# patrikhuber/superviseddescent

Measured on NVIDIA H100. Metric: faces/sec RCR 22-landmark detect, higher is better.
Workload: dtype f32

## Files before the change

### superviseddescent_b200/csrc/sd_hog.cu

```cuda
#include "sd_internal.cuh"
#include "sd_hog_common.cuh"

#include <cmath>
#include <cuda_pipeline.h>

namespace {

constexpr int kHogThreads = 256;

struct HogArgs {
    const uint8_t* images;
    int width, height, row_stride;
    long long image_stride;
    int image_count;
    const int* image_index;
    const sd_roi* roi;
    const sd_frame* frames;
    uint8_t* roi_miss;
    const float* x;
    long long ldx;
    int N, L;
    int variant, nc, cs, K, fs, dd;
    const int* half;
    HogOrient orient;
    const int* rtab;
    const float* btab;
    int tma_count;
    float* A;
    long long ld;
    int* geometry;
    uint8_t* patches;
    int8_t* bins;
    int* status;
};

__device__ __forceinline__ int clip_index(int x, int a, int b) { return x >= a ? (x < b ? x : b - 1) : a; }
__device__ __forceinline__ short sat_short(int v) { return (short)(v > 32767 ? 32767 : (v < -32768 ? -32768 : v)); }

__global__ void hog_geometry_kernel(const float* __restrict__ x, long long ldx, int N, int L, const sd_eyes_dev eyes, float rel,
                                    int fixed_half, int fs, int* __restrict__ half_out, int* __restrict__ rtab, int* __restrict__ status)
{
    const int i = blockIdx.x;
    if (i >= N) return;
    __shared__ int s_half;
    if (threadIdx.x == 0) {
        bool degenerate;
        const int half = sd_patch_half(x + (long long)i * ldx, L, eyes, rel, fixed_half, &degenerate);
        if (degenerate) atomicOr(status, 1);
        half_out[i] = half;
        s_half = half;
    }
    __syncthreads();
    const int P = 2 * s_half;
    int* rt = rtab + (long long)i * 5 * fs;
    for (int t = threadIdx.x; t < fs; t += blockDim.x) {
        const double inv_scale = __ddiv_rn((double)fs, (double)P);
        const double scale = __ddiv_rn(1.0, inv_scale);
        float f = (float)__dadd_rn(__dmul_rn((double)t + 0.5, scale), -0.5);
        const int s = (int)floorf(f);
        f = __fsub_rn(f, (float)s);
        int sx = s;
        float fx = f;
        if (sx < 0) { fx = 0.f; sx = 0; }
        if (sx >= P - 1) { fx = 0.f; sx = P - 1; }
        const short2 xa = make_short2(sat_short(__float2int_rn(__fmul_rn(__fsub_rn(1.f, fx), 2048.f))),
                                      sat_short(__float2int_rn(__fmul_rn(fx, 2048.f))));
        const short2 yb = make_short2(sat_short(__float2int_rn(__fmul_rn(__fsub_rn(1.f, f), 2048.f))),
                                      sat_short(__float2int_rn(__fmul_rn(f, 2048.f))));
        rt[t] = sx;
        rt[fs + t] = *reinterpret_cast<const int*>(&xa);
        rt[2 * fs + t] = clip_index(s, 0, P);
        rt[3 * fs + t] = clip_index(s + 1, 0, P);
        rt[4 * fs + t] = *reinterpret_cast<const int*>(&yb);
    }
}

__global__ void hog_bintab_kernel(int fs, int nc, int cs, float* __restrict__ btab)
{
    __shared__ int s_sbin[256];
    for (int t = threadIdx.x; t < fs; t += blockDim.x) {
        int b;
        float w1, w2;
        hog_spatial_weight(t, cs, &b, &w1, &w2);
        s_sbin[t] = b;
        for (int c = 0; c < nc; ++c) btab[c * fs + t] = (b == c) ? w1 : ((b == c - 1) ? w2 : 0.f);
    }
    __syncthreads();
    int* lohi = reinterpret_cast<int*>(btab + nc * fs);
    for (int c = threadIdx.x; c < nc; c += blockDim.x) {
        int lo = fs, hi = -1;
        for (int t = 1; t <= fs - 2; ++t) {
            const int b = s_sbin[t];
            if (b == c || b == c - 1) { if (t < lo) lo = t; hi = t; }
        }
        lohi[c] = lo;
        lohi[nc + c] = hi;
    }
}

struct HogSmem {
    int patch, bin, r1, xofs, yofs0, yofs1, xa, yb, wcell, lo, hi, vote, mbar, stage_end, total;
    int tpad;
};

__host__ __device__ inline int align_up(int v, int a) { return (v + a - 1) / a * a; }

__host__ __device__ inline HogSmem hog_smem_layout(int fs, int nc, int K)
{
    HogSmem s;
    int o = 0;
    s.patch = o;
    o = align_up(fs * fs, 16);
    s.xofs = o;   o += fs * 4;
    s.yofs0 = o;  o += fs * 4;
    s.yofs1 = o;  o += fs * 4;
    s.xa = o;     o += fs * 4;
    s.yb = o;     o += fs * 4;
    s.wcell = o;  o += nc * fs * 4;
    s.lo = o;     o += nc * 4;
    s.hi = o;     o += nc * 4;
    s.mbar = align_up(o, 8); o = s.mbar + 8;
    o = align_up(o, 128);
    s.bin = o;    o = align_up(o + fs * fs, 16);
    s.r1 = o;     o = align_up(o + fs * fs * 4, 16);
    s.tpad = align_up((fs - 2) * nc, 32);
    s.vote = o;
    o += 2 * K * s.tpad * 4;
    s.stage_end = o;
    s.total = align_up(o, 16);
    return s;
}

constexpr int kTmaClasses = 8;
__host__ __device__ constexpr int hog_tma_box(int c) { return c == 0 ? 32 : c == 1 ? 48 : c == 2 ? 64 : c == 3 ? 80 : c == 4 ? 96 : c == 5 ? 112 : c == 6 ? 128 : 160; }
struct HogMaps { CUtensorMap m[kTmaClasses]; };

template <int KT, int NCT, int CST, int NT>
__global__ void __launch_bounds__(NT, NCT > 0 ? 2048 / NT : 0) hog_patch_kernel(const __grid_constant__ HogArgs a, const __grid_constant__ HogMaps maps)
{
    static_assert(NT % 32 == 0 && NT >= 64, "hog_patch_kernel needs whole warps and at least 64 threads");
    constexpr int kWarps = NT / 32;
    extern __shared__ __align__(128) unsigned char smem[];
    const int K = KT > 0 ? KT : a.K;
    const int nc = NCT > 0 ? NCT : a.nc;
    const int fs = (NCT > 0 && CST > 0) ? NCT * CST : a.fs;
    const int cells = nc * nc;
    const HogSmem lay = hog_smem_layout(fs, nc, K);
    uint8_t* s_patch = smem + lay.patch;
    int8_t* s_bin = reinterpret_cast<int8_t*>(smem + lay.bin);
    float* s_gmag = reinterpret_cast<float*>(smem + lay.r1);
    int* s_xofs = reinterpret_cast<int*>(smem + lay.xofs);
    int* s_yofs0 = reinterpret_cast<int*>(smem + lay.yofs0);
    int* s_yofs1 = reinterpret_cast<int*>(smem + lay.yofs1);
    short2* s_xa = reinterpret_cast<short2*>(smem + lay.xa);
    short2* s_yb = reinterpret_cast<short2*>(smem + lay.yb);
    float* s_wcell = reinterpret_cast<float*>(smem + lay.wcell);
    int* s_lo = reinterpret_cast<int*>(smem + lay.lo);
    int* s_hi = reinterpret_cast<int*>(smem + lay.hi);
    float* s_T = reinterpret_cast<float*>(smem + lay.vote);
    uint64_t* s_mbar = reinterpret_cast<uint64_t*>(smem + lay.mbar);

    const int tid = threadIdx.x;
    const int lane = tid & 31, warp = tid >> 5;
    const long long patch_id = blockIdx.x;
    const int sample = (int)(patch_id / a.L);
    const int lm = (int)(patch_id - (long long)sample * a.L);

    const float* __restrict__ row = a.x + (long long)sample * a.ldx;
    const int half = __ldg(a.half + sample);
    const int P = 2 * half;
    const int cx = __float2int_rn(row[lm]);
    const int cy = __float2int_rn(row[lm + a.L]);
    int img_idx = a.image_index ? a.image_index[sample] : sample;
    if (img_idx < 0 || img_idx >= a.image_count) {
        img_idx = 0;
        if (tid == 0 && a.status) atomicOr(a.status, 2);
    }
    int W = a.width, H = a.height, rs = a.row_stride;
    const uint8_t* __restrict__ img = a.images + (long long)img_idx * a.image_stride;
    if (a.frames) {
        const sd_frame f = a.frames[img_idx];
        W = f.width; H = f.height; rs = f.row_stride;
        img = a.images + f.offset;
    }
    int rx = 0, ry = 0, rw = W, rh = H;
    if (a.roi) {
        const sd_roi r = a.roi[img_idx];
        rx = r.x; ry = r.y; rw = r.w; rh = r.h; rs = r.row_stride;
        img = a.images + r.offset;
    }
    if (tid == 0 && a.geometry) {
        a.geometry[patch_id * 3 + 0] = cx;
        a.geometry[patch_id * 3 + 1] = cy;
        a.geometry[patch_id * 3 + 2] = half;
    }

    const int x0 = cx - half, y0 = cy - half;
    uint8_t* s_stage = smem + lay.bin;
    const int stage_cap = lay.stage_end - lay.bin;
    int tma_box = 0;
    const int tma_shift = x0 & 15;
#pragma unroll
    for (int c = kTmaClasses - 1; c >= 0; --c)
        if (c < a.tma_count && hog_tma_box(c) >= P + tma_shift && hog_tma_box(c) * hog_tma_box(c) <= stage_cap) tma_box = hog_tma_box(c);
    if (tma_box > 0 && tid == 0) {
        int cls = 0;
#pragma unroll
        for (int c = 0; c < kTmaClasses; ++c) if (hog_tma_box(c) == tma_box) cls = c;
        hog_tma_load(s_mbar, s_stage, &maps.m[cls], x0 - tma_shift, y0, img_idx, tma_box * tma_box);
    }

    {
        const int* __restrict__ rt = a.rtab + (long long)sample * 5 * fs;
        for (int t = tid; t < fs; t += NT) {
            s_xofs[t] = __ldg(rt + t);
            const int xa = __ldg(rt + fs + t), yb = __ldg(rt + 4 * fs + t);
            s_xa[t] = *reinterpret_cast<const short2*>(&xa);
            s_yofs0[t] = __ldg(rt + 2 * fs + t);
            s_yofs1[t] = __ldg(rt + 3 * fs + t);
            s_yb[t] = *reinterpret_cast<const short2*>(&yb);
        }
        for (int i = tid; i < nc * fs; i += NT) s_wcell[i] = __ldg(a.btab + i);
        const int* __restrict__ lohi = reinterpret_cast<const int*>(a.btab + nc * fs);
        if (tid < nc) { s_lo[tid] = __ldg(lohi + tid); s_hi[tid] = __ldg(lohi + nc + tid); }
    }
    {
        const bool resident = x0 >= rx && y0 >= ry && x0 + P <= rx + rw && y0 + P <= ry + rh && x0 >= 0 && y0 >= 0 && x0 + P <= W && y0 + P <= H;
        const uintptr_t align_bits = reinterpret_cast<uintptr_t>(img) | (uintptr_t)rs;
        const bool vec16 = !tma_box && resident && (align_bits & 15) == 0;
        const bool words = !tma_box && resident && (align_bits & 3) == 0;
        const int shiftb = tma_box ? tma_shift : (vec16 ? ((x0 - rx) & 15) : (words ? ((x0 - rx) & 3) : 0));
        const int pitch = tma_box ? tma_box : ((P + 15 + 15) & ~15);
        const bool staged = pitch * P <= stage_cap;
        bool miss = false;
        if (staged) {
            if (tma_box) {
            } else if (vec16) {
                const int nvec = (shiftb + P + 15) >> 4;
                const int gs = nvec <= 8 ? 3 : (nvec <= 16 ? 4 : 5);
                const int lv = lane & ((1 << gs) - 1), lr = lane >> gs, rows_per_pass = 32 >> gs;
                const uint8_t* wrow = img + (long long)(y0 - ry) * rs + (x0 - rx - shiftb);
                for (int r = warp * rows_per_pass + lr; r < P; r += kWarps * rows_per_pass)
                    for (int v = lv; v < nvec; v += (1 << gs))
                        reinterpret_cast<uint4*>(s_stage + r * pitch)[v] = __ldg(reinterpret_cast<const uint4*>(wrow + (long long)r * rs) + v);
            } else if (words) {
                const int nwords = (shiftb + P + 3) >> 2;
                const uint8_t* wrow = img + (long long)(y0 - ry) * rs + (x0 - rx - shiftb);
                for (int r = warp; r < P; r += kWarps) {
                    const uint32_t* src = reinterpret_cast<const uint32_t*>(wrow + (long long)r * rs);
                    uint32_t* dst = reinterpret_cast<uint32_t*>(s_stage + r * pitch);
                    for (int w = lane; w < nwords; w += 32) dst[w] = __ldg(src + w);
                }
            } else {
                for (int r = warp; r < P; r += kWarps) {
                    const int iy = y0 + r;
                    const bool rowin = (unsigned)iy < (unsigned)H;
                    const bool rowres = iy >= ry && iy < ry + rh;
                    for (int c = lane; c < P; c += 32) {
                        const int ix = x0 + c;
                        int v = 0;
                        if (rowin && (unsigned)ix < (unsigned)W) {
                            if (rowres && ix >= rx && ix < rx + rw) v = __ldg(img + (long long)(iy - ry) * rs + (ix - rx));
                            else miss = true;
                        }
                        s_stage[r * pitch + c] = (uint8_t)v;
                    }
                }
            }
            __syncthreads();
            if (tma_box) hog_tma_wait(s_mbar);
            if (fs <= 64) {
                const int groups = NT / fs;
                const int dx = tid % fs, g = tid / fs;
                if (g < groups) {
                    const int sx = s_xofs[dx];
                    const int sx1 = min(sx + 1, P - 1);
                    const int ax = s_xa[dx].x, bx = s_xa[dx].y;
                    const uint8_t* base = s_stage + shiftb;
#pragma unroll 4
                    for (int dy = g; dy < fs; dy += groups) {
                        const short2 yb = s_yb[dy];
                        const uint8_t* r0 = base + s_yofs0[dy] * pitch;
                        const uint8_t* r1 = base + s_yofs1[dy] * pitch;
                        const int t0 = (int)r0[sx] * ax + (int)r0[sx1] * bx;
                        const int t1 = (int)r1[sx] * ax + (int)r1[sx1] * bx;
                        const int v = ((((int)yb.x * (t0 >> 4)) >> 16) + (((int)yb.y * (t1 >> 4)) >> 16) + 2) >> 2;
                        s_patch[dy * fs + dx] = (uint8_t)v;
                    }
                }
            } else {
                for (int dy = warp; dy < fs; dy += kWarps) {
                    const short2 yb = s_yb[dy];
                    const uint8_t* r0 = s_stage + s_yofs0[dy] * pitch + shiftb;
                    const uint8_t* r1 = s_stage + s_yofs1[dy] * pitch + shiftb;
                    for (int dx = lane; dx < fs; dx += 32) {
                        const int sx = s_xofs[dx];
                        const int sx1 = min(sx + 1, P - 1);
                        const short2 xa = s_xa[dx];
                        const int t0 = (int)r0[sx] * xa.x + (int)r0[sx1] * xa.y;
                        const int t1 = (int)r1[sx] * xa.x + (int)r1[sx1] * xa.y;
                        const int v = ((((int)yb.x * (t0 >> 4)) >> 16) + (((int)yb.y * (t1 >> 4)) >> 16) + 2) >> 2;
                        s_patch[dy * fs + dx] = (uint8_t)v;
                    }
                }
            }
        } else {
            __syncthreads();
            for (int dy = warp; dy < fs; dy += kWarps) {
                const short2 yb = s_yb[dy];
                const int iy0 = y0 + s_yofs0[dy], iy1 = y0 + s_yofs1[dy];
                for (int dx = lane; dx < fs; dx += 32) {
                    const int sx = s_xofs[dx];
                    const short2 xa = s_xa[dx];
                    int p[4];
#pragma unroll
                    for (int q = 0; q < 4; ++q) {
                        const int ix = x0 + sx + (q & 1), iy = (q & 2) ? iy1 : iy0;
                        int v = 0;
                        if ((q & 1) && xa.y == 0) { p[q] = 0; continue; }
                        if ((unsigned)ix < (unsigned)W && (unsigned)iy < (unsigned)H) {
                            if (ix >= rx && ix < rx + rw && iy >= ry && iy < ry + rh) v = __ldg(img + (long long)(iy - ry) * rs + (ix - rx));
                            else miss = true;
                        }
                        p[q] = v;
                    }
                    const int t0 = p[0] * xa.x + p[1] * xa.y;
                    const int t1 = p[2] * xa.x + p[3] * xa.y;
                    const int v = ((((int)yb.x * (t0 >> 4)) >> 16) + (((int)yb.y * (t1 >> 4)) >> 16) + 2) >> 2;
                    s_patch[dy * fs + dx] = (uint8_t)v;
                }
            }
        }
        if (miss && a.roi_miss) a.roi_miss[img_idx] = 1;
        if (a.patches) {
            __syncthreads();
            for (int i = tid; i < fs * fs; i += NT) a.patches[patch_id * fs * fs + i] = s_patch[i];
        }
    }
    __syncthreads();

    {
        const int iw = fs - 2, npix = iw * iw;
        for (int i = tid; i < npix; i += NT) {
            const int y = i / iw, x = i - y * iw;
            const int idx = (y + 1) * fs + (x + 1);
            const int gx = (int)s_patch[idx + 1] - (int)s_patch[idx - 1];
            const int gy = (int)s_patch[idx + fs] - (int)s_patch[idx - fs];
            const int g2 = gx * gx + gy * gy;
            const float g = __fsqrt_rn((float)g2);
            const int b = hog_bin(a.orient, K, gx, gy, g);
            s_bin[idx] = (int8_t)b;
            s_gmag[idx] = b < 0 ? 0.f : g;
        }
    }
    if (a.bins) {
        __syncthreads();
        for (int idx = tid; idx < fs * fs; idx += NT) {
            const int y = idx / fs, x = idx - y * fs;
            const bool interior = x >= 1 && x <= fs - 2 && y >= 1 && y <= fs - 2;
            a.bins[patch_id * fs * fs + idx] = interior ? s_bin[idx] : (int8_t)-1;
        }
    }
    if (!a.A) return;
    __syncthreads();

    {
        const int nrow = fs - 2, ntask = nrow * nc, tpad = lay.tpad;
        for (int task = tid; task < ntask; task += NT) {
            const int ci = task / nrow, y = 1 + task - ci * nrow;
            const int xlo = s_lo[ci], xhi = s_hi[ci];
            const int8_t* bp = s_bin + y * fs + xlo;
            const float* gp = s_gmag + y * fs + xlo;
            const float* wp = s_wcell + ci * fs + xlo;
            float* T = s_T + task;
            for (int b = 0; b < 2 * K; ++b) T[b * tpad] = 0.f;
#pragma unroll 2
            for (int x = xlo; x <= xhi; ++x) {
                const int b = max((int)*bp++, 0);
                float* q = T + b * tpad;
                *q = __fadd_rn(*q, __fmul_rn(*gp++, *wp++));
            }
        }
        __syncthreads();
        float* __restrict__ out = a.A + (long long)sample * a.ld + (long long)lm * cells * a.dd;
        for (int i = tid; i < 2 * K * cells; i += NT) {
            const int b = i / cells, c = i - b * cells;
            const int cj = c / nc, ci = c - cj * nc;
            const int ylo = s_lo[cj], yhi = s_hi[cj];
            const float* Tp = s_T + b * tpad + ci * nrow + (ylo - 1);
            const float* wy = s_wcell + cj * fs + ylo;
            float acc = 0.f;
            for (int y = ylo; y <= yhi; ++y) acc = __fadd_rn(acc, __fmul_rn(*Tp++, *wy++));
            out[i] = acc;
        }
    }
}

struct NormArgs {
    float* A;
    long long ld;
    int N, L, nc, K, dd, variant, per_cta;
};

__host__ __device__ inline int hog_norm_smem(int nc, int K, int per_cta)
{
    const int cells = nc * nc;
    return per_cta * (8 + 2 * K * cells * 4 + cells * 8 + (nc + 1) * (nc + 1) * 8);
}

template <int KT>
__global__ void __launch_bounds__(kHogThreads) hog_normalise_kernel(const NormArgs a)
{
    extern __shared__ __align__(16) unsigned char s_norm[];
    const int K = KT > 0 ? KT : a.K;
    const int nc = a.nc, nb = nc + 1, cells = nc * nc, blocks = nb * nb, hsz = 2 * K * cells, per_lm = cells * a.dd;
    const long long first = (long long)blockIdx.x * a.per_cta;
    const int np = (int)min((long long)a.per_cta, (long long)a.N * a.L - first);
    long long* s_slice = reinterpret_cast<long long*>(s_norm);
    double* s_energy = reinterpret_cast<double*>(s_slice + a.per_cta);
    double* s_fac = s_energy + a.per_cta * cells;
    float* s_hist = reinterpret_cast<float*>(s_fac + a.per_cta * blocks);
    for (int p = threadIdx.x; p < np; p += kHogThreads) {
        const long long id = first + p;
        const int sample = (int)(id / a.L), lm = (int)(id - (long long)sample * a.L);
        s_slice[p] = (long long)sample * a.ld + (long long)lm * per_lm;
        if (lm == 0) a.A[(long long)sample * a.ld + (long long)a.L * per_lm] = 1.0f;
    }
    __syncthreads();
    for (int i = threadIdx.x; i < np * hsz; i += kHogThreads) {
        const int p = i / hsz;
        __pipeline_memcpy_async(s_hist + i, a.A + s_slice[p] + (i - p * hsz), sizeof(float));
    }
    __pipeline_commit();
    __pipeline_wait_prior(0);
    __syncthreads();
    for (int i = threadIdx.x; i < np * cells; i += kHogThreads) {
        const int p = i / cells, c = i - p * cells;
        s_energy[i] = (double)hog_cell_energy(s_hist + p * hsz + c, cells, K);
    }
    __syncthreads();
    for (int i = threadIdx.x; i < np * blocks; i += kHogThreads) {
        const int p = i / blocks, j = i - p * blocks;
        const int jy = j / nb, jx = j - jy * nb;
        s_fac[i] = hog_block_factor(s_energy + p * cells, nc, max(jx - 1, 0), min(jx, nc - 1), max(jy - 1, 0), min(jy, nc - 1));
    }
    __syncthreads();
    for (int i = threadIdx.x; i < np * cells; i += kHogThreads) {
        const int p = i / cells, c = i - p * cells;
        const int cj = c / nc, ci = c - cj * nc;
        const double* F = s_fac + p * blocks + cj * nb + ci;
        const double fac[4] = {F[0], F[1], F[nb], F[nb + 1]};
        float* __restrict__ out = a.A + s_slice[p] + ci * nc + cj;
        hog_cell_features(fac, s_hist + p * hsz + c, cells, K, a.variant, [=](int d, float v) { out[d * cells] = v; });
    }
}

int launch_hog(sd_ctx* ctx, const sd_image_batch* images, const int32_t* d_image_index, const float* d_x,
               int64_t ldx, int N, int L, const sd_normalisation* eyes, const sd_hog_param* p, float* d_A,
               int64_t ld, int32_t* d_geometry, uint8_t* d_patches, int8_t* d_bins)
{
    SD_REQUIRE(ctx, images && images->d_data && d_x && p, "null argument");
    SD_REQUIRE(ctx, N >= 0 && L >= 1, "bad sample / landmark count");
    SD_REQUIRE(ctx, p->variant == 0 || p->variant == 1, "unknown HOG variant");
    SD_REQUIRE(ctx, p->num_bins >= 1 && p->num_bins <= SD_MAX_BINS, "num_bins must be in [1,16]");
    SD_REQUIRE(ctx, p->num_cells >= 1 && p->cell_size >= 1, "bad cell configuration");
    const int fs = p->num_cells * p->cell_size;
    SD_REQUIRE(ctx, fs > 3 && fs <= 256, "resized patch must be 4..256 px (hog.c:545-546 asserts > 3)");
    SD_REQUIRE(ctx, (fs + p->cell_size / 2) / p->cell_size == p->num_cells, "hogWidth != num_cells");
    SD_REQUIRE(ctx, ldx >= 2 * L, "ldx < 2L");
    if (N == 0) return SD_OK;
    const bool fixed = !eyes || eyes->kind == 0;
    int fixed_half = 0;
    if (fixed) {
        fixed_half = p->num_cells * (p->cell_size / 2);
        SD_REQUIRE(ctx, 2 * fixed_half == fs, "the fixed-patch HogTransform needs an even cell_size (patch == num_cells * cell_size)");
    } else if (eyes->kind != 1) {
        return sd_fail(ctx, SD_ERR_INVALID, "unknown normalisation kind");
    }

    HogArgs a;
    sd_eyes_dev eyes_dev;
    memset(&eyes_dev, 0, sizeof(eyes_dev));
    int rc = fixed ? SD_OK : sd_eyes_to_dev(ctx, eyes, L, &eyes_dev);
    if (rc) return rc;
    a.images = images->d_data;
    a.width = images->width; a.height = images->height; a.row_stride = images->row_stride;
    a.image_stride = images->image_stride; a.image_count = images->count;
    a.image_index = d_image_index;
    a.roi = images->d_roi;
    a.roi_miss = images->d_roi_miss;
    a.frames = images->d_frames;
    if (!d_image_index) SD_REQUIRE(ctx, images->count >= N, "fewer images than samples and no image index");
    a.x = d_x; a.ldx = ldx; a.N = N; a.L = L;
    a.variant = p->variant; a.nc = p->num_cells; a.cs = p->cell_size; a.K = p->num_bins; a.fs = fs;
    a.dd = p->variant == 1 ? 3 * p->num_bins + 4 : 4 * p->num_bins;
    a.A = d_A; a.ld = ld;
    if (d_A) SD_REQUIRE(ctx, ld >= (int64_t)L * a.nc * a.nc * a.dd + 1, "ld < feature length");
    const HogSmem lay = hog_smem_layout(fs, a.nc, a.K);
    const int cells = a.nc * a.nc;
    NormArgs na;
    na.A = d_A; na.ld = ld; na.N = N; na.L = L; na.nc = a.nc; na.K = a.K; na.dd = a.dd; na.variant = a.variant;
    na.per_cta = cells < kHogThreads ? kHogThreads / cells : 1;
    const int norm_smem = hog_norm_smem(a.nc, a.K, na.per_cta);
    SD_REQUIRE(ctx, lay.total <= 227 * 1024 && norm_smem <= 227 * 1024, "HOG configuration needs more than 227 KB of shared memory");
    const long long blocks = (long long)N * L;
    SD_REQUIRE(ctx, blocks < 2147483647LL, "too many patches for one launch");
    a.geometry = d_geometry; a.patches = d_patches; a.bins = d_bins;
    a.status = reinterpret_cast<int*>(ctx->d_scratch) + 1;

    hog_orientations(a.K, a.orient);

    const size_t geom_bytes = (size_t)N * sizeof(int) + (size_t)N * 5 * fs * sizeof(int) + (size_t)(a.nc * fs + 2 * a.nc) * sizeof(float);
    int* d_half = (int*)sd_workspace(ctx, SD_WS_GEOM, geom_bytes);
    if (!d_half) return SD_ERR_CUDA;
    int* d_rtab = d_half + N;
    float* d_btab = reinterpret_cast<float*>(d_rtab + (size_t)N * 5 * fs);
    hog_geometry_kernel<<<N, 64, 0, ctx->stream>>>(d_x, ldx, N, L, eyes_dev, p->relative_patch_size, fixed_half, fs, d_half, d_rtab, a.status);
    SD_LAUNCH_CHECK(ctx, "hog_geometry_kernel");
    hog_bintab_kernel<<<1, 256, 0, ctx->stream>>>(fs, a.nc, a.cs, d_btab);
    SD_LAUNCH_CHECK(ctx, "hog_bintab_kernel");
    a.half = d_half;
    a.rtab = d_rtab;
    a.btab = d_btab;

    HogMaps maps;
    memset(&maps, 0, sizeof(maps));
    a.tma_count = 0;
    if (!images->d_roi && (images->image_stride % 16) == 0 && (images->count == 1 || images->image_stride > 0)) {
        for (int c = 0; c < kTmaClasses && hog_tma_box(c) <= 256; ++c) {
            if (!hog_frame_map(images, hog_tma_box(c), hog_tma_box(c), &maps.m[c])) break;
            a.tma_count = c + 1;
        }
    }

    auto kern = hog_patch_kernel<0, 0, 0, kHogThreads>;
    int threads = kHogThreads;
    if (a.K == 4) kern = hog_patch_kernel<4, 0, 0, kHogThreads>;
    else if (a.K == 9) kern = hog_patch_kernel<9, 0, 0, kHogThreads>;
    if (a.nc == 5 && (a.K == 4 || a.K == 9)) {
#define SD_HOG_PICK(KK, CC, TT) if (a.K == KK && a.cs == CC) { kern = hog_patch_kernel<KK, 5, CC, TT>; threads = TT; }
        SD_HOG_PICK(4, 11, 224) SD_HOG_PICK(4, 10, 160) SD_HOG_PICK(4, 8, 160) SD_HOG_PICK(4, 6, 128)
        SD_HOG_PICK(9, 11, 256) SD_HOG_PICK(9, 10, 160) SD_HOG_PICK(9, 8, 160) SD_HOG_PICK(9, 6, 128)
#undef SD_HOG_PICK
    }
    SD_CUDA(ctx, cudaFuncSetAttribute(kern, cudaFuncAttributeMaxDynamicSharedMemorySize, lay.total));
    kern<<<(unsigned)blocks, threads, lay.total, ctx->stream>>>(a, maps);
    SD_LAUNCH_CHECK(ctx, "hog_patch_kernel");
    if (!d_A) return SD_OK;
    auto norm = a.K == 4 ? hog_normalise_kernel<4> : a.K == 9 ? hog_normalise_kernel<9> : hog_normalise_kernel<0>;
    SD_CUDA(ctx, cudaFuncSetAttribute(norm, cudaFuncAttributeMaxDynamicSharedMemorySize, norm_smem));
    norm<<<(unsigned)sd_div_up(blocks, na.per_cta), kHogThreads, norm_smem, ctx->stream>>>(na);
    SD_LAUNCH_CHECK(ctx, "hog_normalise_kernel");
    return SD_OK;
}

}

namespace {
__global__ void bgr2gray_kernel(const uint8_t* __restrict__ bgr, int width, int height, long long srow, long long simg, int count,
                                uint8_t* __restrict__ gray, long long drow, long long dimg, int vec_ok)
{
    const int groups = (width + 3) >> 2;
    const long long total = (long long)count * height * groups;
    for (long long t = blockIdx.x * (long long)blockDim.x + threadIdx.x; t < total; t += (long long)gridDim.x * blockDim.x) {
        const int g = (int)(t % groups);
        const long long ry = t / groups;
        const int y = (int)(ry % height);
        const long long im = ry / height;
        const uint8_t* s = bgr + im * simg + (long long)y * srow + 12 * g;
        uint8_t* d = gray + im * dimg + (long long)y * drow + 4 * g;
        const int x0 = 4 * g;
        if (vec_ok && x0 + 4 <= width) {
            const uint32_t w0 = *reinterpret_cast<const uint32_t*>(s), w1 = *reinterpret_cast<const uint32_t*>(s + 4),
                           w2 = *reinterpret_cast<const uint32_t*>(s + 8);
            const uint32_t b0 = w0 & 255, g0 = (w0 >> 8) & 255, r0 = (w0 >> 16) & 255, b1 = w0 >> 24;
            const uint32_t g1 = w1 & 255, r1 = (w1 >> 8) & 255, b2 = (w1 >> 16) & 255, g2 = w1 >> 24;
            const uint32_t r2 = w2 & 255, b3 = (w2 >> 8) & 255, g3 = (w2 >> 16) & 255, r3 = w2 >> 24;
            const uint32_t y0 = sd_bgr_to_gray(b0, g0, r0), y1 = sd_bgr_to_gray(b1, g1, r1);
            const uint32_t y2 = sd_bgr_to_gray(b2, g2, r2), y3 = sd_bgr_to_gray(b3, g3, r3);
            *reinterpret_cast<uint32_t*>(d) = y0 | (y1 << 8) | (y2 << 16) | (y3 << 24);
        } else {
            for (int k = 0; k < 4 && x0 + k < width; ++k) d[k] = (uint8_t)sd_bgr_to_gray(s[3 * k], s[3 * k + 1], s[3 * k + 2]);
        }
    }
}
}

extern "C" {

int sd_hog_feature_length(int num_landmarks, const sd_hog_param* p)
{
    if (!p) return -1;
    const int dd = p->variant == 1 ? 3 * p->num_bins + 4 : 4 * p->num_bins;
    return num_landmarks * p->num_cells * p->num_cells * dd + 1;
}

int sd_hog_batch(sd_ctx* ctx, const sd_image_batch* images, const int32_t* d_image_index, const float* d_x,
                 int64_t ldx, int num_samples, int num_landmarks, const sd_normalisation* eyes,
                 const sd_hog_param* p, float* d_A, int64_t ld)
{
    if (!ctx) return SD_ERR_INVALID;
    if (num_samples == 0) return SD_OK;
    SD_REQUIRE(ctx, d_A, "null output");
    return launch_hog(ctx, images, d_image_index, d_x, ldx, num_samples, num_landmarks, eyes, p, d_A, ld,
                      nullptr, nullptr, nullptr);
}

int sd_hog_debug(sd_ctx* ctx, const sd_image_batch* images, const int32_t* d_image_index, const float* d_x,
                 int64_t ldx, int num_samples, int num_landmarks, const sd_normalisation* eyes,
                 const sd_hog_param* p, int32_t* d_geometry, uint8_t* d_patches, int8_t* d_bins)
{
    if (!ctx) return SD_ERR_INVALID;
    return launch_hog(ctx, images, d_image_index, d_x, ldx, num_samples, num_landmarks, eyes, p, nullptr, 0,
                      d_geometry, d_patches, d_bins);
}

int sd_bgr2gray(sd_ctx* ctx, const uint8_t* d_bgr, int width, int height, int64_t bgr_row_stride, int64_t bgr_image_stride,
                int count, uint8_t* d_gray, int64_t gray_row_stride, int64_t gray_image_stride)
{
    if (!ctx) return SD_ERR_INVALID;
    SD_REQUIRE(ctx, count >= 0 && width > 0 && height > 0, "bad argument");
    if (count == 0) return SD_OK;
    SD_REQUIRE(ctx, d_bgr && d_gray && bgr_row_stride >= 3LL * width && gray_row_stride >= width, "bad argument");
    const int vec_ok = ((reinterpret_cast<uintptr_t>(d_bgr) | reinterpret_cast<uintptr_t>(d_gray) | (uintptr_t)bgr_row_stride |
                         (uintptr_t)bgr_image_stride | (uintptr_t)gray_row_stride | (uintptr_t)gray_image_stride) & 3) == 0;
    const long long total = (long long)count * height * ((width + 3) >> 2);
    const int blocks = (int)(sd_div_up(total, 256) < 16LL * ctx->sm_count ? sd_div_up(total, 256) : 16LL * ctx->sm_count);
    bgr2gray_kernel<<<blocks, 256, 0, ctx->stream>>>(d_bgr, width, height, bgr_row_stride, bgr_image_stride, count, d_gray,
                                                     gray_row_stride, gray_image_stride, vec_ok);
    SD_LAUNCH_CHECK(ctx, "bgr2gray_kernel");
    return SD_OK;
}

}
```

Baseline: 735,100.

## Pack resize tables, vectorize bilinear resize and gradient stages with byte ops

Merges the per-row/column resize offset tables into a single int4 table and pads the patch, bin and magnitude buffers to word-aligned pitches. The resize loop now produces two output pixels per thread using 32-bit shared loads, __byte_perm and __dp2a, with a scalar fallback for wide offsets. The gradient stage processes four pixels per item from packed words and writes bins as one 32-bit store. The aim is fewer shared-memory transactions and instructions in the resize and gradient phases, in exchange for more complex indexing and a small shared-memory footprint change.

New measurement: 812,600, median of 6. 10.5% higher.

```diff
diff --git a/superviseddescent_b200/csrc/sd_hog.cu b/superviseddescent_b200/csrc/sd_hog.cu
--- a/superviseddescent_b200/csrc/sd_hog.cu
+++ b/superviseddescent_b200/csrc/sd_hog.cu
@@ -98,8 +98,17 @@
     }
 }
 
+__device__ __forceinline__ int hog_resize_out(int yb, int t0, int t1)
+{
+    return (((((int)(short)yb) * (t0 >> 4)) >> 16) + (((yb >> 16) * (t1 >> 4)) >> 16) + 2) >> 2;
+}
+
+__device__ __forceinline__ int byte_of(unsigned lo, unsigned hi, int n) { return (int)(((n < 4 ? lo : hi) >> (8 * (n & 3))) & 0xffu); }
+
 struct HogSmem {
-    int patch, bin, r1, xofs, yofs0, yofs1, xa, yb, wcell, lo, hi, vote, mbar, stage_end, total;
+    int patch, bin, r1, tab, xa, wcell, lo, hi, vote, mbar, stage_end, total;
+    int pp;
+    int pb, pm;
     int tpad;
 };
 
@@ -108,14 +117,15 @@
 __host__ __device__ inline HogSmem hog_smem_layout(int fs, int nc, int K)
 {
     HogSmem s;
+    s.pp = align_up(fs, 4);
+    s.pm = align_up(fs - 2, 4) + 1;
+    s.pb = s.pm - 1;
+    if ((s.pb & 7) == 0 && (fs - 2) * (s.pb + 4) <= fs * fs) s.pb += 4;
     int o = 0;
     s.patch = o;
-    o = align_up(fs * fs, 16);
-    s.xofs = o;   o += fs * 4;
-    s.yofs0 = o;  o += fs * 4;
-    s.yofs1 = o;  o += fs * 4;
+    o = align_up(s.pp * fs, 16);
+    s.tab = o;    o += fs * 16;
     s.xa = o;     o += fs * 4;
-    s.yb = o;     o += fs * 4;
     s.wcell = o;  o += nc * fs * 4;
     s.lo = o;     o += nc * 4;
     s.hi = o;     o += nc * 4;
@@ -127,7 +137,7 @@
     s.vote = o;
     o += 2 * K * s.tpad * 4;
     s.stage_end = o;
-    s.total = align_up(o, 16);
+    s.total = align_up(o + 8, 16);
     return s;
 }
 
@@ -146,14 +156,12 @@
     const int fs = (NCT > 0 && CST > 0) ? NCT * CST : a.fs;
     const int cells = nc * nc;
     const HogSmem lay = hog_smem_layout(fs, nc, K);
+    const int pp = lay.pp, pb = lay.pb, pm = lay.pm;
     uint8_t* s_patch = smem + lay.patch;
     int8_t* s_bin = reinterpret_cast<int8_t*>(smem + lay.bin);
     float* s_gmag = reinterpret_cast<float*>(smem + lay.r1);
-    int* s_xofs = reinterpret_cast<int*>(smem + lay.xofs);
-    int* s_yofs0 = reinterpret_cast<int*>(smem + lay.yofs0);
-    int* s_yofs1 = reinterpret_cast<int*>(smem + lay.yofs1);
+    int4* s_tab = reinterpret_cast<int4*>(smem + lay.tab);
     short2* s_xa = reinterpret_cast<short2*>(smem + lay.xa);
-    short2* s_yb = reinterpret_cast<short2*>(smem + lay.yb);
     float* s_wcell = reinterpret_cast<float*>(smem + lay.wcell);
     int* s_lo = reinterpret_cast<int*>(smem + lay.lo);
     int* s_hi = reinterpret_cast<int*>(smem + lay.hi);
@@ -213,12 +221,9 @@
     {
         const int* __restrict__ rt = a.rtab + (long long)sample * 5 * fs;
         for (int t = tid; t < fs; t += NT) {
-            s_xofs[t] = __ldg(rt + t);
-            const int xa = __ldg(rt + fs + t), yb = __ldg(rt + 4 * fs + t);
+            const int xa = __ldg(rt + fs + t);
             s_xa[t] = *reinterpret_cast<const short2*>(&xa);
-            s_yofs0[t] = __ldg(rt + 2 * fs + t);
-            s_yofs1[t] = __ldg(rt + 3 * fs + t);
-            s_yb[t] = *reinterpret_cast<const short2*>(&yb);
+            s_tab[t] = make_int4(__ldg(rt + t), __ldg(rt + 2 * fs + t), __ldg(rt + 3 * fs + t), __ldg(rt + 4 * fs + t));
         }
         for (int i = tid; i < nc * fs; i += NT) s_wcell[i] = __ldg(a.btab + i);
         const int* __restrict__ lohi = reinterpret_cast<const int*>(a.btab + nc * fs);
@@ -241,6 +246,7 @@
                 const int lv = lane & ((1 << gs) - 1), lr = lane >> gs, rows_per_pass = 32 >> gs;
                 const uint8_t* wrow = img + (long long)(y0 - ry) * rs + (x0 - rx - shiftb);
                 for (int r = warp * rows_per_pass + lr; r < P; r += kWarps * rows_per_pass)
+#pragma unroll 1
                     for (int v = lv; v < nvec; v += (1 << gs))
                         reinterpret_cast<uint4*>(s_stage + r * pitch)[v] = __ldg(reinterpret_cast<const uint4*>(wrow + (long long)r * rs) + v);
             } else if (words) {
@@ -249,6 +255,7 @@
                 for (int r = warp; r < P; r += kWarps) {
                     const uint32_t* src = reinterpret_cast<const uint32_t*>(wrow + (long long)r * rs);
                     uint32_t* dst = reinterpret_cast<uint32_t*>(s_stage + r * pitch);
+#pragma unroll 1
                     for (int w = lane; w < nwords; w += 32) dst[w] = __ldg(src + w);
                 }
             } else {
@@ -270,47 +277,64 @@
             __syncthreads();
             if (tma_box) hog_tma_wait(s_mbar);
             if (fs <= 64) {
-                const int groups = NT / fs;
-                const int dx = tid % fs, g = tid / fs;
+                const int np = (fs + 1) >> 1, groups = NT / np;
+                const int j = tid % np, g = tid / np;
                 if (g < groups) {
-                    const int sx = s_xofs[dx];
-                    const int sx1 = min(sx + 1, P - 1);
-                    const int ax = s_xa[dx].x, bx = s_xa[dx].y;
-                    const uint8_t* base = s_stage + shiftb;
-#pragma unroll 4
-                    for (int dy = g; dy < fs; dy += groups) {
-                        const short2 yb = s_yb[dy];
-                        const uint8_t* r0 = base + s_yofs0[dy] * pitch;
-                        const uint8_t* r1 = base + s_yofs1[dy] * pitch;
-                        const int t0 = (int)r0[sx] * ax + (int)r0[sx1] * bx;
-                        const int t1 = (int)r1[sx] * ax + (int)r1[sx1] * bx;
-                        const int v = ((((int)yb.x * (t0 >> 4)) >> 16) + (((int)yb.y * (t1 >> 4)) >> 16) + 2) >> 2;
-                        s_patch[dy * fs + dx] = (uint8_t)v;
+                    const int dxa = 2 * j, dxb = min(dxa + 1, fs - 1);
+                    const int sxa = s_tab[dxa].x, sxb = s_tab[dxb].x;
+                    const unsigned xa = *reinterpret_cast<const unsigned*>(s_xa + dxa), xb = *reinterpret_cast<const unsigned*>(s_xa + dxb);
+                    const int q = (shiftb + sxa) & ~3;
+                    const int oa = shiftb + sxa - q, ob = shiftb + sxb - q;
+                    uint8_t* out = s_patch + dxa;
+                    if (ob <= 6) {
+                        const unsigned sa = oa | (oa + 1) << 4, sb = ob | (ob + 1) << 4;
+                        const uint8_t* base = s_stage + q;
+#pragma unroll 2
+                        for (int dy = g; dy < fs; dy += groups) {
+                            const int4 yt = s_tab[dy];
+                            const unsigned* r0 = reinterpret_cast<const unsigned*>(base + yt.y * pitch);
+                            const unsigned* r1 = reinterpret_cast<const unsigned*>(base + yt.z * pitch);
+                            const unsigned a0 = r0[0], a1 = r0[1], b0 = r1[0], b1 = r1[1];
+                            const int va = hog_resize_out(yt.w, __dp2a_lo(xa, __byte_perm(a0, a1, sa), 0u), __dp2a_lo(xa, __byte_perm(b0, b1, sa), 0u));
+                            const int vb = hog_resize_out(yt.w, __dp2a_lo(xb, __byte_perm(a0, a1, sb), 0u), __dp2a_lo(xb, __byte_perm(b0, b1, sb), 0u));
+                            *reinterpret_cast<uint16_t*>(out + dy * pp) = (uint16_t)(va | vb << 8);
+                        }
+                    } else {
+                        const int ax = s_xa[dxa].x, bx = s_xa[dxa].y, cx = s_xa[dxb].x, dx = s_xa[dxb].y;
+                        const int sxa1 = min(sxa + 1, P - 1), sxb1 = min(sxb + 1, P - 1);
+                        const uint8_t* base = s_stage + shiftb;
+                        for (int dy = g; dy < fs; dy += groups) {
+                            const int4 yt = s_tab[dy];
+                            const uint8_t* r0 = base + yt.y * pitch;
+                            const uint8_t* r1 = base + yt.z * pitch;
+                            const int va = hog_resize_out(yt.w, (int)r0[sxa] * ax + (int)r0[sxa1] * bx, (int)r1[sxa] * ax + (int)r1[sxa1] * bx);
+                            const int vb = hog_resize_out(yt.w, (int)r0[sxb] * cx + (int)r0[sxb1] * dx, (int)r1[sxb] * cx + (int)r1[sxb1] * dx);
+                            *reinterpret_cast<uint16_t*>(out + dy * pp) = (uint16_t)(va | vb << 8);
+                        }
                     }
                 }
             } else {
                 for (int dy = warp; dy < fs; dy += kWarps) {
-                    const short2 yb = s_yb[dy];
-                    const uint8_t* r0 = s_stage + s_yofs0[dy] * pitch + shiftb;
-                    const uint8_t* r1 = s_stage + s_yofs1[dy] * pitch + shiftb;
+                    const int4 yt = s_tab[dy];
+                    const uint8_t* r0 = s_stage + yt.y * pitch + shiftb;
+                    const uint8_t* r1 = s_stage + yt.z * pitch + shiftb;
                     for (int dx = lane; dx < fs; dx += 32) {
-                        const int sx = s_xofs[dx];
+                        const int sx = s_tab[dx].x;
                         const int sx1 = min(sx + 1, P - 1);
                         const short2 xa = s_xa[dx];
                         const int t0 = (int)r0[sx] * xa.x + (int)r0[sx1] * xa.y;
                         const int t1 = (int)r1[sx] * xa.x + (int)r1[sx1] * xa.y;
-                        const int v = ((((int)yb.x * (t0 >> 4)) >> 16) + (((int)yb.y * (t1 >> 4)) >> 16) + 2) >> 2;
-                        s_patch[dy * fs + dx] = (uint8_t)v;
+                        s_patch[dy * pp + dx] = (uint8_t)hog_resize_out(yt.w, t0, t1);
                     }
                 }
             }
         } else {
             __syncthreads();
             for (int dy = warp; dy < fs; dy += kWarps) {
-                const short2 yb = s_yb[dy];
-                const int iy0 = y0 + s_yofs0[dy], iy1 = y0 + s_yofs1[dy];
+                const int4 yt = s_tab[dy];
+                const int iy0 = y0 + yt.y, iy1 = y0 + yt.z;
                 for (int dx = lane; dx < fs; dx += 32) {
-                    const int sx = s_xofs[dx];
+                    const int sx = s_tab[dx].x;
                     const short2 xa = s_xa[dx];
                     int p[4];
 #pragma unroll
@@ -326,31 +350,41 @@
                     }
                     const int t0 = p[0] * xa.x + p[1] * xa.y;
                     const int t1 = p[2] * xa.x + p[3] * xa.y;
-                    const int v = ((((int)yb.x * (t0 >> 4)) >> 16) + (((int)yb.y * (t1 >> 4)) >> 16) + 2) >> 2;
-                    s_patch[dy * fs + dx] = (uint8_t)v;
+                    s_patch[dy * pp + dx] = (uint8_t)hog_resize_out(yt.w, t0, t1);
                 }
             }
         }
         if (miss && a.roi_miss) a.roi_miss[img_idx] = 1;
         if (a.patches) {
             __syncthreads();
-            for (int i = tid; i < fs * fs; i += NT) a.patches[patch_id * fs * fs + i] = s_patch[i];
+            for (int i = tid; i < fs * fs; i += NT) {
+                const int y = i / fs;
+                a.patches[patch_id * fs * fs + i] = s_patch[y * pp + (i - y * fs)];
+            }
         }
     }
     __syncthreads();
 
     {
-        const int iw = fs - 2, npix = iw * iw;
-        for (int i = tid; i < npix; i += NT) {
-            const int y = i / iw, x = i - y * iw;
-            const int idx = (y + 1) * fs + (x + 1);
-            const int gx = (int)s_patch[idx + 1] - (int)s_patch[idx - 1];
-            const int gy = (int)s_patch[idx + fs] - (int)s_patch[idx - fs];
-            const int g2 = gx * gx + gy * gy;
-            const float g = __fsqrt_rn((float)g2);
-            const int b = hog_bin(a.orient, K, gx, gy, g);
-            s_bin[idx] = (int8_t)b;
-            s_gmag[idx] = b < 0 ? 0.f : g;
+        const int iw = fs - 2, runs = (iw + 3) >> 2, nitem = iw * runs;
+        const int pw = pp >> 2;
+        for (int i = tid; i < nitem; i += NT) {
+            const int y = i / runs, r = i - y * runs;
+            const unsigned* c = reinterpret_cast<const unsigned*>(s_patch) + (y + 1) * pw + r;
+            const unsigned c0 = c[0], c1 = c[1], u0 = c[-pw], u1 = c[1 - pw], d0 = c[pw], d1 = c[pw + 1];
+            unsigned bins = 0;
+            float* gm = s_gmag + y * pm + 4 * r;
+#pragma unroll
+            for (int k = 0; k < 4; ++k) {
+                const int gx = byte_of(c0, c1, k + 2) - byte_of(c0, c1, k);
+                const int gy = byte_of(d0, d1, k + 1) - byte_of(u0, u1, k + 1);
+                const int g2 = gx * gx + gy * gy;
+                const float g = __fsqrt_rn((float)g2);
+                const int b = hog_bin(a.orient, K, gx, gy, g);
+                bins |= (unsigned)(b & 0xff) << (8 * k);
+                gm[k] = b < 0 ? 0.f : g;
+            }
+            *reinterpret_cast<unsigned*>(s_bin + y * pb + 4 * r) = bins;
         }
     }
     if (a.bins) {
@@ -358,7 +392,7 @@
         for (int idx = tid; idx < fs * fs; idx += NT) {
             const int y = idx / fs, x = idx - y * fs;
             const bool interior = x >= 1 && x <= fs - 2 && y >= 1 && y <= fs - 2;
-            a.bins[patch_id * fs * fs + idx] = interior ? s_bin[idx] : (int8_t)-1;
+            a.bins[patch_id * fs * fs + idx] = interior ? s_bin[(y - 1) * pb + x - 1] : (int8_t)-1;
         }
     }
     if (!a.A) return;
@@ -369,8 +403,8 @@
         for (int task = tid; task < ntask; task += NT) {
             const int ci = task / nrow, y = 1 + task - ci * nrow;
             const int xlo = s_lo[ci], xhi = s_hi[ci];
-            const int8_t* bp = s_bin + y * fs + xlo;
-            const float* gp = s_gmag + y * fs + xlo;
+            const int8_t* bp = s_bin + (y - 1) * pb + (xlo - 1);
+            const float* gp = s_gmag + (y - 1) * pm + (xlo - 1);
             const float* wp = s_wcell + ci * fs + xlo;
             float* T = s_T + task;
             for (int b = 0; b < 2 * K; ++b) T[b * tpad] = 0.f;
```
